# Makiato1999/HRI-EMO

Measured on AMD Instinct MI355X. Metric: utterances/sec fwd+bwd, d=768 T_a=400 T_t=128 N_e=6, higher is better.
Workload: dtype bf16; 1 GPU; FusionWithEmotionDecoder fwd+bwd (train mode, dropout 0.1), d=768 T_a=400 T_t=128 N_e=6 H=8, 2 fusion + 2 decoder layers, all-False masks (BASELINE cfg2); global_batch=64, batch_per_gpu=64, parallelism=dp1, grad_allreduce=none, launch=hipGraph replay, streams=2

## Files before the change

hri-emo_amd/csrc/attention.hip:

```cpp
#include <stdlib.h>

#include <type_traits>

#include "common.h"

struct AttnArgs {
  const bf16_t *Q, *K, *V;
  long ldq, ldk, ldv;
  bf16_t* O; long ldo;
  const bf16_t* dO; long lddo;
  bf16_t *dQ, *dK, *dV;
  long lddq, lddk, lddv;
  const uint8_t* kpm;
  float* lse;
  float* delta;
  float* probs;
  float* csq;
  float* cskv;
  int B, H, Lq, Lk;
  float scale;
  uint32_t thr16; float inv_keep; uint64_t seed; uint32_t site; int b_offset;
  float l2ik, keepfrac;
  const unsigned long long* seed_dev;
  unsigned long long* mbits;
// ... 1 lines not shown
  const int* cu_k;
  uint8_t* Oq; long ldoq;
  uint8_t* So; long ldso;
};

__device__ __forceinline__ AttnArgs localize(const AttnArgs& a0, int b, int h) {
  AttnArgs a = a0;
  if (a0.cu_q != nullptr) {
    const int q0 = a0.cu_q[b], k0 = a0.cu_k[b];
    const int Lq = a0.cu_q[b + 1] - q0, Lk = a0.cu_k[b + 1] - k0;
    const long sq = (long)q0 - (long)b * Lq, sk = (long)k0 - (long)b * Lk;
    a.Q += sq * a.ldq;
    if (a.O != nullptr) a.O += sq * a.ldo;
    if (a.dO != nullptr) a.dO += sq * a.lddo;
    if (a.dQ != nullptr) a.dQ += sq * a.lddq;
    a.K += sk * a.ldk;
    a.V += sk * a.ldv;
    if (a.dK != nullptr) a.dK += sk * a.lddk;
    if (a.dV != nullptr) a.dV += sk * a.lddv;
    const long bh = (long)b * a.H + h;
    if (a.lse != nullptr) a.lse += bh * (a0.Lq - Lq);
    if (a.delta != nullptr) a.delta += bh * (a0.Lq - Lq);
    if (a.mbits != nullptr) a.mbits += bh * ((long)a0.Lq * ((a0.Lk + 63) >> 6) - (long)Lq * ((Lk + 63) >> 6));
    a.Lq = Lq; a.Lk = Lk;
    a.kpm = nullptr;
  }
  return a;
}

#define EXP2(x) __builtin_amdgcn_exp2f(x)
#define LOG2E 1.4426950408889634f
#define LN2 0.6931471805599453f

template <int HD> struct AttnGeom {
  static constexpr int HDP = (HD + 31) / 32 * 32;
  static constexpr int KS = HDP / 32;
  static constexpr int DT = HD / 16;
  static constexpr int STRIDE = HDP * 2 + 32;
  static constexpr int CH = HD / 8;
  static constexpr int CHP = HDP / 8;
};

__device__ __forceinline__ bf16x8 zero8() {
  bf16x8 z;
#pragma unroll
  for (int i = 0; i < 8; ++i) z[i] = (bf16_t)0.f;
  return z;
}

__device__ __forceinline__ bf16x8 tr_frag(const char* tile, int stride, int row0, int col0, int lane) {
  const int g = lane >> 4, i = lane & 15;
  const char* a0 = tile + (row0 + 4 * g + (i >> 2)) * stride + (col0 + 4 * (i & 3)) * 2;
  s16x4 lo = __builtin_amdgcn_ds_read_tr16_b64_v4i16((LDS_PTR(s16x4))a0);
  s16x4 hi = __builtin_amdgcn_ds_read_tr16_b64_v4i16((LDS_PTR(s16x4))(a0 + 16 * stride));
  typedef __attribute__((ext_vector_type(8))) short s16x8;
  s16x8 r = {lo[0], lo[1], lo[2], lo[3], hi[0], hi[1], hi[2], hi[3]};
  return __builtin_bit_cast(bf16x8, r);
}
__device__ __forceinline__ bf16x8 row_frag(const char* tile, int stride, int row, int chunk) {
  return *(LDS_PTR(const bf16x8))(tile + row * stride + chunk * 16);
}

template <int HD, int NR, int NT>
__device__ __forceinline__ void load_tile(char* tile, const bf16_t* base, long ld, int row_first, int nrows_total, int tid) {
  using G = AttnGeom<HD>;
  for (int id = tid; id < NR * G::CHP; id += NT) {
// ... 22 lines not shown
    const u32x4_t v = __builtin_amdgcn_raw_buffer_load_b128(rsrc, ok ? (int)((r * ld + c * 8) * 2) : (int)0x80000000u, 0, 0);
    t.v[k] = __builtin_bit_cast(bf16x8, v);
  }
}
template <int HD, int NR, int NT>
__device__ __forceinline__ void tile_commit(const TileRegs<HD, NR, NT>& t, char* tile, int tid) {
  using G = AttnGeom<HD>;
#pragma unroll
  for (int k = 0; k < TileRegs<HD, NR, NT>::NPT; ++k) {
    const int id = tid + k * NT;
    const int r = id / G::CHP, c = id - r * G::CHP;
    if (id < NR * G::CHP) *(LDS_PTR(bf16x8))(tile + r * G::STRIDE + c * 16) = t.v[k];
  }
}

#ifndef DKV_QT
#define DKV_QT 32
#endif

__device__ __forceinline__ void tile_and_head(int ntiles, int nbh, int& tile, int& bh, int l = blockIdx.x) {
  const int full = (nbh >> 3) << 3;
  const int lim = full * ntiles;
  if (l < lim) {
    const int r = l >> 3;
    tile = r % ntiles;
    bh = (r / ntiles) * 8 + (l & 7);
  } else {
    const int r = l - lim;
    tile = r % ntiles;
    bh = full + r / ntiles;
  }
}

template <int HD, int NW, int QW, bool WB>
__global__ __launch_bounds__(NW * 64) void attn_fwd_kernel(const AttnArgs a0) {
  using G = AttnGeom<HD>;
  constexpr int KS = G::KS, DT = G::DT, STRIDE = G::STRIDE, NT = NW * 64;
  __shared__ __attribute__((aligned(16))) char lds[2 * 64 * STRIDE + 64 * 4 + 16];
  char* Kt = lds;
  char* Vt = lds + 64 * STRIDE;
  float* mb = (float*)(lds + 2 * 64 * STRIDE);
  int* padflag = (int*)(lds + 2 * 64 * STRIDE + 64 * 4);

  const int tid = threadIdx.x, lane = tid & 63, wave = tid >> 6, g = lane >> 4, i = lane & 15;
  int tile, bh;
  tile_and_head((a0.Lq + NW * QW * 16 - 1) / (NW * QW * 16), a0.B * a0.H, tile, bh);
  const int b = bh / a0.H, h = bh - b * a0.H;
  const AttnArgs a = localize(a0, b, h);
  if (tile * (NW * QW * 16) >= a.Lq) return;
  const int qbase = tile * (NW * QW * 16) + wave * QW * 16;

  bf16x8 qf[QW][KS];
#pragma unroll
  for (int qs = 0; qs < QW; ++qs) {
    const int qc = min(qbase + qs * 16 + i, a.Lq - 1);
    const bf16_t* qp = a.Q + ((long)b * a.Lq + qc) * a.ldq + h * HD;
#pragma unroll
    for (int ks = 0; ks < KS; ++ks) {
      const int e = ks * 32 + 8 * g;
      qf[qs][ks] = (e < HD) ? *(const bf16x8*)(qp + e) : zero8();
    }
  }
  f32x4 o[QW][DT];
  float m[QW], l[QW];
#pragma unroll
  for (int qs = 0; qs < QW; ++qs) {
    m[qs] = -INFINITY; l[qs] = 0.f;
#pragma unroll
    for (int dt = 0; dt < DT; ++dt) o[qs][dt] = (f32x4){0.f, 0.f, 0.f, 0.f};
  }
  const float sl2 = a.scale * LOG2E;
  const uint32_t key32 = site_key(eff_seed(a.seed, a.seed_dev), a.site, (uint32_t)((a.b_offset + b) * a.H + h));
  const bf16_t* Kb = a.K + (long)b * a.Lk * a.ldk + h * HD;
  const bf16_t* Vb = a.V + (long)b * a.Lk * a.ldv + h * HD;
  const int nkt = (a.Lk + 63) >> 6;

  constexpr bool PF = true;
  TileRegs<HD, 64, NT> kr, vr;
  if (PF) {
    tile_fetch<HD, 64, NT>(kr, Kb, a.ldk, 0, a.Lk, tid);
    tile_fetch<HD, 64, NT>(vr, Vb, a.ldv, 0, a.Lk, tid);
  }
  for (int kt = 0; kt < nkt; ++kt) {
    __syncthreads();
    if (PF) {
      tile_commit<HD, 64, NT>(kr, Kt, tid);
      tile_commit<HD, 64, NT>(vr, Vt, tid);
    } else {
      load_tile<HD, 64, NT>(Kt, Kb, a.ldk, kt * 64, a.Lk, tid);
      load_tile<HD, 64, NT>(Vt, Vb, a.ldv, kt * 64, a.Lk, tid);
    }
    if (tid < 64) {
      const int key = kt * 64 + tid;
      const bool pad = key >= a.Lk || (a.kpm != nullptr && a.kpm[(long)b * a.Lk + key] != 0);
      mb[tid] = pad ? -INFINITY : 0.f;
      const bool anyp = __builtin_amdgcn_ballot_w64(pad) != 0;
      if (tid == 0) padflag[0] = anyp ? 1 : 0;
    }
    __syncthreads();
    if (PF && kt + 1 < nkt) {
      tile_fetch<HD, 64, NT>(kr, Kb, a.ldk, (kt + 1) * 64, a.Lk, tid);
      tile_fetch<HD, 64, NT>(vr, Vb, a.ldv, (kt + 1) * 64, a.Lk, tid);
    }

    f32x4 s[QW][4];
#pragma unroll
    for (int qs = 0; qs < QW; ++qs)
#pragma unroll
      for (int n = 0; n < 4; ++n) s[qs][n] = (f32x4){0.f, 0.f, 0.f, 0.f};
#pragma unroll
    for (int n = 0; n < 4; ++n)
#pragma unroll
      for (int ks = 0; ks < KS; ++ks) {
        const bf16x8 kf = row_frag(Kt, STRIDE, n * 16 + i, ks * 4 + g);
#pragma unroll
        for (int qs = 0; qs < QW; ++qs) s[qs][n] = __builtin_amdgcn_mfma_f32_16x16x32_bf16(kf, qf[qs][ks], s[qs][n], 0, 0, 0);
      }

    const bool has_pad = padflag[0] != 0;
#pragma unroll
    for (int qs = 0; qs < QW; ++qs) {
      float mx = -INFINITY;
      if (has_pad) {
#pragma unroll
        for (int n = 0; n < 4; ++n) {
          const f32x4 bias = *(LDS_PTR(const f32x4))(mb + n * 16 + 4 * g);
#pragma unroll
          for (int r = 0; r < 4; ++r) s[qs][n][r] += bias[r];
        }
      }
#pragma unroll
      for (int n = 0; n < 4; ++n)
#pragma unroll
        for (int r = 0; r < 4; ++r) mx = fmaxf(mx, s[qs][n][r]);
      mx = fmaxf(mx, __shfl_xor(mx, 16));
      mx = fmaxf(mx, __shfl_xor(mx, 32));
      mx *= sl2;
      const float mnew = fmaxf(m[qs], mx);
      if (__builtin_amdgcn_ballot_w64(mnew > m[qs] + 8.f) != 0) {
        const float ms = (mnew == -INFINITY) ? 0.f : mnew;
        const float alpha = EXP2(m[qs] - ms);
        m[qs] = mnew;
        l[qs] *= alpha;
#pragma unroll
        for (int dt = 0; dt < DT; ++dt) o[qs][dt] *= alpha;
      }
      const float nm = (m[qs] == -INFINITY) ? 0.f : -m[qs];
      float rs = 0.f;
#pragma unroll
      for (int n = 0; n < 4; ++n)
#pragma unroll
        for (int r = 0; r < 4; ++r) {
          const float p = EXP2(fmaf(s[qs][n][r], sl2, nm));
          s[qs][n][r] = p;
          rs += p;
        }
      rs += __shfl_xor(rs, 16);
      rs += __shfl_xor(rs, 32);
      l[qs] += rs;
      if (a.thr16 != 0) {
        const uint32_t hb = drop_base(key32, (uint32_t)(qbase + qs * 16 + i), (uint32_t)((kt * 64 + 4 * g) >> 1));
        uint32_t bits = 0u;
#pragma unroll
        for (int n = 0; n < 4; ++n)
#pragma unroll
          for (int pr = 0; pr < 2; ++pr) {
            const uint32_t x = mix24(hb + (uint32_t)(n * 8 + pr) * DROP_CB);
            const bool k0 = keep_lo(x, a.thr16), k1 = keep_hi(x, a.thr16);
            s[qs][n][2 * pr] = k0 ? s[qs][n][2 * pr] : 0.f;
            s[qs][n][2 * pr + 1] = k1 ? s[qs][n][2 * pr + 1] : 0.f;
            if (WB) bits |= (k0 ? 1u : 0u) << (n * 4 + 2 * pr) | (k1 ? 1u : 0u) << (n * 4 + 2 * pr + 1);
          }
        if (WB && qbase + qs * 16 + i < a.Lq)
          ((unsigned short*)(a.mbits + (((long)bh * a.Lq + qbase + qs * 16 + i) * nkt + kt)))[g] = (unsigned short)bits;
      }
    }

#pragma unroll
    for (int s2 = 0; s2 < 2; ++s2) {
      bf16x8 pf[QW];
#pragma unroll
      for (int qs = 0; qs < QW; ++qs)
#pragma unroll
        for (int j = 0; j < 8; ++j) pf[qs][j] = (bf16_t)s[qs][2 * s2 + (j >> 2)][j & 3];
#pragma unroll
      for (int dt = 0; dt < DT; ++dt) {
        const bf16x8 vf = tr_frag(Vt, STRIDE, 32 * s2, dt * 16, lane);
#pragma unroll
        for (int qs = 0; qs < QW; ++qs) o[qs][dt] = __builtin_amdgcn_mfma_f32_16x16x32_bf16(vf, pf[qs], o[qs][dt], 0, 0, 0);
      }
    }
  }

#pragma unroll
  for (int qs = 0; qs < QW; ++qs) {
    const int q = qbase + qs * 16 + i;
    if (q >= a.Lq) continue;
    const float inv = (a.thr16 != 0 ? a.inv_keep : 1.f) / l[qs];
    bf16_t* op = a.O + ((long)b * a.Lq + q) * a.ldo + h * HD + 4 * g;
#pragma unroll
    for (int dt = 0; dt < DT; ++dt) {
      bf16x4 w;
#pragma unroll
      for (int r = 0; r < 4; ++r) w[r] = (bf16_t)(o[qs][dt][r] * inv);
      *(bf16x4*)(op + dt * 16) = w;
    }
    if (g == 0 && a.lse != nullptr) a.lse[((long)b * a.H + h) * a.Lq + q] = (m[qs] + log2f(l[qs])) * LN2;
  }
  if constexpr (DT % 2 == 0) {
    if (a.Oq != nullptr) {
#pragma unroll
      for (int qs = 0; qs < QW; ++qs) {
        const int q = qbase + qs * 16 + i;
        const float inv = (a.thr16 != 0 ? a.inv_keep : 1.f) / l[qs];
        const long row = (long)b * a.Lq + min(q, a.Lq - 1);
#pragma unroll
        for (int kb = 0; kb < DT / 2; ++kb) {
          float f[8];
          float amax = 0.f;
#pragma unroll
          for (int j = 0; j < 8; ++j) {
            f[j] = (float)(bf16_t)(o[qs][2 * kb + (j >> 2)][j & 3] * inv);
            amax = fmaxf(amax, fabsf(f[j]));
          }
          amax = fmaxf(amax, __shfl_xor(amax, 16));
// ... 82 lines not shown
        const bf16x8 ov = *(const bf16x8*)(op + e);
#pragma unroll
        for (int j = 0; j < 8; ++j) part += (float)dof[qs][ks][j] * (float)ov[j];
      } else {
        qf[qs][ks] = zero8();
        dof[qs][ks] = zero8();
      }
    }
    part += __shfl_xor(part, 16);
    part += __shfl_xor(part, 32);
    dl[qs] = part;
    const long li = ((long)b * a.H + h) * a.Lq + qc;
    lse2[qs] = a.lse[li] * LOG2E;
    if (g == 0 && q < a.Lq) a.delta[li] = part;
  }
  f32x4 dq[QW][DT];
#pragma unroll
  for (int qs = 0; qs < QW; ++qs)
#pragma unroll
    for (int dt = 0; dt < DT; ++dt) dq[qs][dt] = (f32x4){0.f, 0.f, 0.f, 0.f};

  const float sl2 = a.scale * LOG2E;
  float cexp[QW], dlk[QW];
#pragma unroll
  for (int qs = 0; qs < QW; ++qs) {
    cexp[qs] = (a.thr16 != 0 ? log2f(a.inv_keep) : 0.f) - lse2[qs];
    dlk[qs] = a.thr16 != 0 ? dl[qs] / a.inv_keep : dl[qs];
  }
  const uint32_t key32 = site_key(eff_seed(a.seed, a.seed_dev), a.site, (uint32_t)((a.b_offset + b) * a.H + h));
  const bf16_t* Kb = a.K + (long)b * a.Lk * a.ldk + h * HD;
  const bf16_t* Vb = a.V + (long)b * a.Lk * a.ldv + h * HD;
  const int nkt = (a.Lk + 63) >> 6;

  constexpr bool PF = (NW == 4);
  TileRegs<HD, 64, NT> kr, vr;
  if (PF) {
    tile_fetch<HD, 64, NT>(kr, Kb, a.ldk, 0, a.Lk, tid);
    tile_fetch<HD, 64, NT>(vr, Vb, a.ldv, 0, a.Lk, tid);
  }
  for (int kt = 0; kt < nkt; ++kt) {
    __syncthreads();
    if (PF) {
      tile_commit<HD, 64, NT>(kr, Kt, tid);
      tile_commit<HD, 64, NT>(vr, Vt, tid);
    } else {
      load_tile<HD, 64, NT>(Kt, Kb, a.ldk, kt * 64, a.Lk, tid);
      load_tile<HD, 64, NT>(Vt, Vb, a.ldv, kt * 64, a.Lk, tid);
    }
    if (tid < 64) {
      const int key = kt * 64 + tid;
      const bool pad = key >= a.Lk || (a.kpm != nullptr && a.kpm[(long)b * a.Lk + key] != 0);
      mb[tid] = pad ? -INFINITY : 0.f;
    }
    __syncthreads();
    if (PF && kt + 1 < nkt) {
      tile_fetch<HD, 64, NT>(kr, Kb, a.ldk, (kt + 1) * 64, a.Lk, tid);
      tile_fetch<HD, 64, NT>(vr, Vb, a.ldv, (kt + 1) * 64, a.Lk, tid);
    }

    f32x4 s[QW][4], dp[QW][4];
#pragma unroll
    for (int qs = 0; qs < QW; ++qs)
#pragma unroll
      for (int n = 0; n < 4; ++n) {
        s[qs][n] = (f32x4){0.f, 0.f, 0.f, 0.f};
        dp[qs][n] = (f32x4){0.f, 0.f, 0.f, 0.f};
      }
#pragma unroll
    for (int n = 0; n < 4; ++n)
#pragma unroll
      for (int ks = 0; ks < KS; ++ks) {
        const bf16x8 kf = row_frag(Kt, STRIDE, n * 16 + i, ks * 4 + g);
        const bf16x8 vf = row_frag(Vt, STRIDE, n * 16 + i, ks * 4 + g);
#pragma unroll
        for (int qs = 0; qs < QW; ++qs) {
          s[qs][n] = __builtin_amdgcn_mfma_f32_16x16x32_bf16(kf, qf[qs][ks], s[qs][n], 0, 0, 0);
          dp[qs][n] = __builtin_amdgcn_mfma_f32_16x16x32_bf16(vf, dof[qs][ks], dp[qs][n], 0, 0, 0);
        }
      }
#pragma unroll
    for (int qs = 0; qs < QW; ++qs) {
      const uint32_t hb = drop_base(key32, (uint32_t)(qbase + qs * 16 + i), (uint32_t)((kt * 64 + 4 * g) >> 1));
      uint32_t bits = 0xffffu;
      constexpr bool from_bits = BITS;
      if (from_bits && a.thr16 != 0)
        bits = ((const unsigned short*)(a.mbits + (((long)bh * a.Lq + min(qbase + qs * 16 + i, a.Lq - 1)) * nkt + kt)))[g];
#pragma unroll
      for (int n = 0; n < 4; ++n) {
        const f32x4 bias = *(LDS_PTR(const f32x4))(mb + n * 16 + 4 * g);
#pragma unroll
        for (int pr = 0; pr < 2; ++pr) {
          uint32_t x = 0xffffffffu;
          if (a.thr16 != 0 && !from_bits) x = mix24(hb + (uint32_t)(n * 8 + pr) * DROP_CB);
#pragma unroll
          for (int e = 0; e < 2; ++e) {
            const int r = 2 * pr + e;
            const float pk = EXP2(fmaf(s[qs][n][r], sl2, bias[r] + cexp[qs]));
            float dpd = dp[qs][n][r];
            if (a.thr16 != 0) {
              const bool keep = from_bits ? ((bits >> (n * 4 + r)) & 1u) != 0u : (e ? keep_hi(x, a.thr16) : keep_lo(x, a.thr16));
              dpd = keep ? dpd : 0.f;
            }
            s[qs][n][r] = pk * (dpd - dlk[qs]);
          }
        }
      }
    }
#pragma unroll
    for (int s2 = 0; s2 < 2; ++s2) {
      bf16x8 dsf[QW];
#pragma unroll
      for (int qs = 0; qs < QW; ++qs)
#pragma unroll
        for (int j = 0; j < 8; ++j) dsf[qs][j] = (bf16_t)s[qs][2 * s2 + (j >> 2)][j & 3];
#pragma unroll
      for (int dt = 0; dt < DT; ++dt) {
        const bf16x8 ktf = tr_frag(Kt, STRIDE, 32 * s2, dt * 16, lane);
#pragma unroll
        for (int qs = 0; qs < QW; ++qs) dq[qs][dt] = __builtin_amdgcn_mfma_f32_16x16x32_bf16(ktf, dsf[qs], dq[qs][dt], 0, 0, 0);
      }
    }
  }
  f32x4 cs[DT];
#pragma unroll
  for (int dt = 0; dt < DT; ++dt) cs[dt] = (f32x4){0.f, 0.f, 0.f, 0.f};
#pragma unroll
  for (int qs = 0; qs < QW; ++qs) {
    const int q = qbase + qs * 16 + i;
    if (q >= a.Lq) continue;
    bf16_t* dqp = a.dQ + ((long)b * a.Lq + q) * a.lddq + h * HD + 4 * g;
#pragma unroll
    for (int dt = 0; dt < DT; ++dt) {
      bf16x4 w;
#pragma unroll
      for (int r = 0; r < 4; ++r) {
        const float v = dq[qs][dt][r] * a.scale;
        w[r] = (bf16_t)v;
        cs[dt][r] += v;
      }
      *(bf16x4*)(dqp + dt * 16) = w;
    }
  }
  if (a.csq != nullptr) {
    __syncthreads();
    block_colsum_store<DT, NW>(cs, (float*)lds, csq_row, tid);
  }
}

template <int HD, bool BITS>
__global__ __launch_bounds__(512) void attn_bwd_qres_kernel(const AttnArgs a0) {
  using G = AttnGeom<HD>;
  constexpr int KS = G::KS, DT = G::DT, STRIDE = G::STRIDE, NW = 8, NT = 512, NQ = 128, KT = 64;
  constexpr int PS = KT * 2 + 32;
  __shared__ __attribute__((aligned(16))) char lds[2 * NQ * STRIDE + 2 * KT * STRIDE + 2 * NQ * PS + KT * 4];
  char* const Qi = lds;
// ... 184 lines not shown
      }
      *(bf16x4*)(dqp + dt * 16) = w;
    }
  }
  float* red = (float*)lds;
  if (a.csq != nullptr) {
    block_colsum_store<DT, NW>(csq, red, a.csq + (long)b * ((long)a.H * HD) + h * HD, tid);
    __syncthreads();
  }
  if (a.cskv != nullptr) {
#pragma unroll
    for (int dt = 0; dt < DT; ++dt) {
      f32x4 v = cs[dt];
#pragma unroll
      for (int m = 1; m < 16; m <<= 1) {
#pragma unroll
        for (int r = 0; r < 4; ++r) v[r] += __shfl_xor(v[r], m, 64);
      }
      if (i == 0) *(f32x4*)(red + wave * (DT * 16) + dt * 16 + 4 * g) = v;
    }
    __syncthreads();
    float* row = a.cskv + (long)b * (2L * a.H * HD) + h * HD;
    for (int c = tid; c < 2 * DT * 16; c += NT) {
      const int wh = c / (DT * 16), e = c - wh * (DT * 16);
      float t = 0.f;
#pragma unroll
      for (int w = 0; w < 4; ++w) t += red[(2 * w + (wh == 0 ? 1 : 0)) * (DT * 16) + e];
      row[(long)wh * a.H * HD + e] = t;
    }
  }
}

template <int HD, int NW, int KW, int QT>
__global__ __launch_bounds__(NW * 64) void attn_bwd_dkv_hash_kernel(const AttnArgs a0) {
  using G = AttnGeom<HD>;
  constexpr int KS = G::KS, DT = G::DT, STRIDE = G::STRIDE, NT = NW * 64;
  static_assert(QT == 32 || QT == 64, "query tile");
  constexpr int NQS = QT / 16, NKQ = QT / 32;
  constexpr int TILE_BYTES = 2 * QT * STRIDE + 2 * QT * 4;
  __shared__ __attribute__((aligned(16))) char lds[2 * TILE_BYTES];
  const int tid = threadIdx.x, lane = tid & 63, wave = tid >> 6, g = lane >> 4, i = lane & 15;
  int tile, bh;
  tile_and_head((a0.Lk + NW * KW * 16 - 1) / (NW * KW * 16), a0.B * a0.H, tile, bh);
  const int b = bh / a0.H, h = bh - b * a0.H;
  const AttnArgs a = localize(a0, b, h);
  float* const cskv_row = a.cskv != nullptr ? a.cskv + (long)(b * gridDim_tiles(a0.Lk, NW * KW * 16) + tile) * (2L * a.H * HD) + h * HD : nullptr;
  if (tile * (NW * KW * 16) >= a.Lk) {
    if (cskv_row != nullptr) for (int e = tid; e < HD; e += NT) { cskv_row[e] = 0.f; cskv_row[(long)a.H * HD + e] = 0.f; }
    return;
  }
  const int kbase = tile * (NW * KW * 16) + wave * KW * 16;

  bf16x8 kreg[KW][KS], vreg[KW][KS];
  bool kvalid[KW];
#pragma unroll
  for (int kw = 0; kw < KW; ++kw) {
    const int key = kbase + kw * 16 + i;
    const int kc = min(key, a.Lk - 1);
    kvalid[kw] = key < a.Lk && !(a.kpm != nullptr && a.kpm[(long)b * a.Lk + kc] != 0);
    const bf16_t* kp = a.K + ((long)b * a.Lk + kc) * a.ldk + h * HD;
    const bf16_t* vp = a.V + ((long)b * a.Lk + kc) * a.ldv + h * HD;
#pragma unroll
    for (int ks = 0; ks < KS; ++ks) {
      const int e = ks * 32 + 8 * g;
      kreg[kw][ks] = (e < HD) ? *(const bf16x8*)(kp + e) : zero8();
      vreg[kw][ks] = (e < HD) ? *(const bf16x8*)(vp + e) : zero8();
    }
// ... 10 lines not shown
      dv[kw][dt] = (f32x4){0.f, 0.f, 0.f, 0.f};
    }
  const float sl2 = a.scale * LOG2E;
  const uint32_t key32 = site_key(eff_seed(a.seed, a.seed_dev), a.site, (uint32_t)((a.b_offset + b) * a.H + h));
#pragma unroll
  for (int kw = 0; kw < KW; ++kw) hkb[kw] = drop_base(key32, 0u, (uint32_t)((kbase + kw * 16 + i) >> 1));
  const bf16_t* Qb = a.Q + (long)b * a.Lq * a.ldq + h * HD;
  const bf16_t* dOb = a.dO + (long)b * a.Lq * a.lddo + h * HD;
  const long lbase = ((long)b * a.H + h) * a.Lq;
  const int nqt = (a.Lq + QT - 1) / QT;

  const float l2ik = a.thr16 != 0 ? log2f(a.inv_keep) : 0.f, keepfrac = a.thr16 != 0 ? 1.f / a.inv_keep : 1.f;
  constexpr bool PF = (NW == 4);
  TileRegs<HD, QT, NT> qr, dor;
  float lse_r = 0.f, del_r = 0.f;
  auto fetch = [&](int qt) {
    tile_fetch<HD, QT, NT>(qr, Qb, a.ldq, qt * QT, a.Lq, tid);
    tile_fetch<HD, QT, NT>(dor, dOb, a.lddo, qt * QT, a.Lq, tid);
    if (tid < QT) {
      const int q = qt * QT + tid;
      lse_r = q < a.Lq ? l2ik - a.lse[lbase + q] * LOG2E : -INFINITY;
      del_r = q < a.Lq ? a.delta[lbase + q] * keepfrac : 0.f;
    }
  };
  auto commit = [&](int buf) {
    char* base = lds + buf * TILE_BYTES;
    tile_commit<HD, QT, NT>(qr, base, tid);
    tile_commit<HD, QT, NT>(dor, base + QT * STRIDE, tid);
    if (tid < QT) {
      ((float*)(base + 2 * QT * STRIDE))[tid] = lse_r;
      ((float*)(base + 2 * QT * STRIDE))[QT + tid] = del_r;
    }
  };
  fetch(0);
  commit(0);
  if (nqt > 1) fetch(1);
  __syncthreads();
  for (int qt = 0; qt < nqt; ++qt) {
    const char* Qt = lds + (qt & 1) * TILE_BYTES;
    const char* dOt = Qt + QT * STRIDE;
    const float* lse_s = (const float*)(Qt + 2 * QT * STRIDE);
    const float* del_s = lse_s + QT;
    if (qt + 1 < nqt) {
      commit((qt + 1) & 1);
      if (qt + 2 < nqt) fetch(qt + 2);
    }

    f32x4 s[KW][NQS], dp[KW][NQS];
#pragma unroll
    for (int kw = 0; kw < KW; ++kw)
#pragma unroll
      for (int qs = 0; qs < NQS; ++qs) {
        s[kw][qs] = (f32x4){0.f, 0.f, 0.f, 0.f};
        dp[kw][qs] = (f32x4){0.f, 0.f, 0.f, 0.f};
      }
#pragma unroll
    for (int qs = 0; qs < NQS; ++qs)
#pragma unroll
      for (int ks = 0; ks < KS; ++ks) {
        const bf16x8 qfr = row_frag(Qt, STRIDE, qs * 16 + i, ks * 4 + g);
        const bf16x8 dofr = row_frag(dOt, STRIDE, qs * 16 + i, ks * 4 + g);
#pragma unroll
        for (int kw = 0; kw < KW; ++kw) {
          s[kw][qs] = __builtin_amdgcn_mfma_f32_16x16x32_bf16(qfr, kreg[kw][ks], s[kw][qs], 0, 0, 0);
          dp[kw][qs] = __builtin_amdgcn_mfma_f32_16x16x32_bf16(dofr, vreg[kw][ks], dp[kw][qs], 0, 0, 0);
        }
      }
    bf16x8 pf[KW][NKQ], dsf[KW][NKQ];
#pragma unroll
    for (int qs = 0; qs < NQS; ++qs) {
      const f32x4 lse4 = *(LDS_PTR(const f32x4))(lse_s + qs * 16 + 4 * g);
      const f32x4 del4 = *(LDS_PTR(const f32x4))(del_s + qs * 16 + 4 * g);
#pragma unroll
      for (int kw = 0; kw < KW; ++kw) {
        const uint32_t key = (uint32_t)(kbase + kw * 16 + i);
#pragma unroll
        for (int r = 0; r < 4; ++r) {
          const float pk = kvalid[kw] ? EXP2(fmaf(s[kw][qs][r], sl2, lse4[r])) : 0.f;
          float pd = pk, dpd = dp[kw][qs][r];
          if (a.thr16 != 0) {
            const uint32_t x = mix24(hkb[kw] + (uint32_t)(qt * QT + qs * 16 + 4 * g + r) * DROP_CA);
            const bool keep = (key & 1u) ? keep_hi(x, a.thr16) : keep_lo(x, a.thr16);
            pd = keep ? pk : 0.f;
            dpd = keep ? dpd : 0.f;
          }
          pf[kw][qs >> 1][(qs & 1) * 4 + r] = (bf16_t)pd;
          dsf[kw][qs >> 1][(qs & 1) * 4 + r] = (bf16_t)(pk * (dpd - del4[r]));
        }
      }
    }
#pragma unroll
    for (int kq = 0; kq < NKQ; ++kq)
#pragma unroll
      for (int dt = 0; dt < DT; ++dt) {
        const bf16x8 dotf = tr_frag(dOt, STRIDE, 32 * kq, dt * 16, lane);
        const bf16x8 qtf = tr_frag(Qt, STRIDE, 32 * kq, dt * 16, lane);
#pragma unroll
        for (int kw = 0; kw < KW; ++kw) {
          dv[kw][dt] = __builtin_amdgcn_mfma_f32_16x16x32_bf16(dotf, pf[kw][kq], dv[kw][dt], 0, 0, 0);
          dk[kw][dt] = __builtin_amdgcn_mfma_f32_16x16x32_bf16(qtf, dsf[kw][kq], dk[kw][dt], 0, 0, 0);
        }
      }
    __syncthreads();
  }
  f32x4 csk[DT], csv[DT];
#pragma unroll
  for (int dt = 0; dt < DT; ++dt) { csk[dt] = (f32x4){0.f, 0.f, 0.f, 0.f}; csv[dt] = (f32x4){0.f, 0.f, 0.f, 0.f}; }
#pragma unroll
  for (int kw = 0; kw < KW; ++kw) {
    const int key = kbase + kw * 16 + i;
    if (key >= a.Lk) continue;
    bf16_t* dkp = a.dK + ((long)b * a.Lk + key) * a.lddk + h * HD + 4 * g;
    bf16_t* dvp = a.dV + ((long)b * a.Lk + key) * a.lddv + h * HD + 4 * g;
#pragma unroll
    for (int dt = 0; dt < DT; ++dt) {
      bf16x4 wk, wv;
#pragma unroll
      for (int r = 0; r < 4; ++r) {
        const float vk = dk[kw][dt][r] * a.scale, vv = dv[kw][dt][r];
        wk[r] = (bf16_t)vk;
        wv[r] = (bf16_t)vv;
        csk[dt][r] += vk;
        csv[dt][r] += vv;
      }
      *(bf16x4*)(dkp + dt * 16) = wk;
      *(bf16x4*)(dvp + dt * 16) = wv;
    }
  }
  if (a.cskv != nullptr) {
    float* row = cskv_row;
    __syncthreads();
    block_colsum_store<DT, NW>(csk, (float*)lds, row, tid);
    block_colsum_store<DT, NW>(csv, (float*)lds + NW * DT * 16, row + (long)a.H * HD, tid);
  }
}

template <int HD, int NW, int KW, int QT, bool BITS, bool FUSED, bool PACKED = false>
// ... 446 lines not shown
  HRIEMO_CHECK(hd == 16 || hd == 32 || hd == 64 || hd == 96 || hd == 128, "attn: head_dim %d not built (16/32/64/96/128)", hd);
  return 0;
}
static int check_common(const AttnArgs& a, int hd) {
  if (check_shape(a.B, a.H, a.Lq, a.Lk, hd)) return 1;
  HRIEMO_CHECK(a.ldq % 8 == 0 && a.ldk % 8 == 0 && a.ldv % 8 == 0, "attn: leading dims must be multiples of 8");
  HRIEMO_CHECK(((uintptr_t)a.Q % 16) == 0 && ((uintptr_t)a.K % 16) == 0 && ((uintptr_t)a.V % 16) == 0, "attn: unaligned Q/K/V");
  return 0;
}
static int check_packed(const AttnArgs& a) {
  HRIEMO_CHECK((a.cu_q == nullptr) == (a.cu_k == nullptr), "attn: cu_seqlens_q and cu_seqlens_k must be given together");
  HRIEMO_CHECK(a.cu_q == nullptr || a.kpm == nullptr, "attn: packed sequences carry their lengths, a key_padding_mask cannot be combined with them");
  return 0;
}

extern "C" int hriemo_attn_plan(int B, int H, int Lq, int Lk, int head_dim, int cus, int* fwd_rows, int* bwd_form, int* dq_rows,
                                int* dkv_rows, int* dq_colsum_rows, int* kv_colsum_rows) {
  HRIEMO_CHECK(fwd_rows != nullptr && bwd_form != nullptr && dq_rows != nullptr && dkv_rows != nullptr && dq_colsum_rows != nullptr &&
                   kv_colsum_rows != nullptr, "attn_plan: bad arguments");
  if (check_shape(B, H, Lq, Lk, head_dim)) return 1;
  const AttnPlan p = attn_plan(B, H, Lq, Lk, head_dim, cus);
  *fwd_rows = p.fwd_rows; *bwd_form = p.bwd_form; *dq_rows = p.dq_rows; *dkv_rows = p.dkv_rows;
  *dq_colsum_rows = p.dq_colsum_rows; *kv_colsum_rows = p.kv_colsum_rows;
  return 0;
}
extern "C" int hriemo_attn_bwd_single_pass(int B, int H, int Lk, int head_dim) { return attn_plan(B, H, 1, Lk, head_dim, 0).bwd_form == 1; }
extern "C" int hriemo_attn_bwd_single_pass_q(int B, int H, int Lq, int Lk, int head_dim) { return attn_plan(B, H, Lq, Lk, head_dim, 0).bwd_form != 0; }
extern "C" int hriemo_attn_bwd_kv_colsum_rows(int B, int H, int Lq, int Lk, int head_dim) { return attn_plan(B, H, Lq, Lk, head_dim, 0).kv_colsum_rows; }
extern "C" int hriemo_attn_bwd_colsum_rows(int B, int H, int L, int head_dim) { return attn_plan(B, H, 1, L, head_dim, 0).kv_colsum_rows; }
extern "C" int hriemo_attn_bwd_dq_colsum_rows(int B, int H, int Lq, int Lk, int head_dim) { return attn_plan(B, H, Lq, Lk, head_dim, 0).dq_colsum_rows; }

extern "C" long hriemo_attn_mask_bytes(int B, int H, int Lq, int Lk) { return (long)B * H * Lq * ((Lk + 63) / 64) * 8; }

template <int N> using Int = std::integral_constant<int, N>;
template <class F> static void with_head_dim(int head_dim, F&& f) {
  switch (head_dim) {
    case 16: f(Int<16>{}); break;
    case 32: f(Int<32>{}); break;
    case 64: f(Int<64>{}); break;
    case 96: f(Int<96>{}); break;
    case 128: f(Int<128>{}); break;
  }
}
template <class F> static void with_tile(int rows, F&& f) {
  if (rows == 128) f(Int<4>{}, Int<2>{});
  else if (rows == 64) f(Int<4>{}, Int<1>{});
  else f(Int<1>{}, Int<1>{});
}
template <class F> static void with_bool(bool v, F&& f) {
  if (v) f(std::true_type{});
  else f(std::false_type{});
}

static void fill_drop(AttnArgs& a, float p, uint64_t seed, const unsigned long long* seed_dev, uint32_t site, int b_offset) {
  DropCfg d = make_drop(p, seed, site);
  a.thr16 = d.thr16; a.inv_keep = d.inv_keep; a.seed = seed; a.site = site; a.b_offset = b_offset; a.seed_dev = seed_dev;
  a.l2ik = d.thr16 != 0 ? log2f(d.inv_keep) : 0.f;
  a.keepfrac = d.thr16 != 0 ? 1.f / d.inv_keep : 1.f;
}
static AttnArgs attn_args(const void* Q, long ldq, const void* K, long ldk, const void* V, long ldv, const unsigned char* key_padding_mask,
                          const float* lse, int B, int H, int Lq, int Lk, int head_dim, float p_drop, unsigned long long seed,
                          const unsigned long long* seed_dev, unsigned site, int b_offset) {
  AttnArgs a = {};
  a.Q = (const bf16_t*)Q; a.K = (const bf16_t*)K; a.V = (const bf16_t*)V;
  a.ldq = ldq; a.ldk = ldk; a.ldv = ldv;
  a.kpm = key_padding_mask; a.lse = (float*)lse; a.B = B; a.H = H; a.Lq = Lq; a.Lk = Lk;
  a.scale = 1.0f / sqrtf((float)head_dim);
// ... 177 lines not shown
```

Before: 8711 utterances/s.

## Specialize attention kernels for partial query/key tiles and set waves-per-EU hints

Attention fwd, bwd-dq and bwd-dkv kernels now split the inner loop into a full-tile path and a tail path instantiated at compile time. The tail path skips MFMA work on key or query sub-blocks past the sequence end, and waves whose rows fall entirely out of range only take part in the shared-memory staging and barriers. The forward and dkv kernels also gain amdgpu_waves_per_eu occupancy hints for some configurations. This trims wasted matrix work on ragged tiles (T_a=400 and T_t=128 are not all multiples of 64), at the cost of more code paths and possible register-pressure or code-size changes.

```diff
diff --git a/hri-emo_amd/csrc/attention.hip b/hri-emo_amd/csrc/attention.hip
--- a/hri-emo_amd/csrc/attention.hip
+++ b/hri-emo_amd/csrc/attention.hip
@@ -57,6 +57,8 @@
 #define LOG2E 1.4426950408889634f
 #define LN2 0.6931471805599453f
 
+template <int N> using Int = std::integral_constant<int, N>;
+
 template <int HD> struct AttnGeom {
   static constexpr int HDP = (HD + 31) / 32 * 32;
   static constexpr int KS = HDP / 32;
@@ -145,8 +147,14 @@
   }
 }
 
+template <int HD, int NW, int QW, bool WB> constexpr int fwd_waves() {
+  if (!WB) return 1;
+  if (NW == 1) return HD == 96 ? 2 : 1;
+  if (QW == 1 && HD == 16) return 6;
+  return ((QW == 1 && HD == 128) || (QW == 2 && HD == 64)) ? 3 : 1;
+}
 template <int HD, int NW, int QW, bool WB>
-__global__ __launch_bounds__(NW * 64) void attn_fwd_kernel(const AttnArgs a0) {
+__global__ __launch_bounds__(NW * 64) __attribute__((amdgpu_waves_per_eu(fwd_waves<HD, NW, QW, WB>()))) void attn_fwd_kernel(const AttnArgs a0) {
   using G = AttnGeom<HD>;
   constexpr int KS = G::KS, DT = G::DT, STRIDE = G::STRIDE, NT = NW * 64;
   __shared__ __attribute__((aligned(16))) char lds[2 * 64 * STRIDE + 64 * 4 + 16];
@@ -188,64 +196,48 @@
   const bf16_t* Vb = a.V + (long)b * a.Lk * a.ldv + h * HD;
   const int nkt = (a.Lk + 63) >> 6;
 
-  constexpr bool PF = true;
-  TileRegs<HD, 64, NT> kr, vr;
-  if (PF) {
-    tile_fetch<HD, 64, NT>(kr, Kb, a.ldk, 0, a.Lk, tid);
-    tile_fetch<HD, 64, NT>(vr, Vb, a.ldv, 0, a.Lk, tid);
-  }
-  for (int kt = 0; kt < nkt; ++kt) {
-    __syncthreads();
-    if (PF) {
-      tile_commit<HD, 64, NT>(kr, Kt, tid);
-      tile_commit<HD, 64, NT>(vr, Vt, tid);
-    } else {
-      load_tile<HD, 64, NT>(Kt, Kb, a.ldk, kt * 64, a.Lk, tid);
-      load_tile<HD, 64, NT>(Vt, Vb, a.ldv, kt * 64, a.Lk, tid);
-    }
-    if (tid < 64) {
-      const int key = kt * 64 + tid;
-      const bool pad = key >= a.Lk || (a.kpm != nullptr && a.kpm[(long)b * a.Lk + key] != 0);
-      mb[tid] = pad ? -INFINITY : 0.f;
-      const bool anyp = __builtin_amdgcn_ballot_w64(pad) != 0;
-      if (tid == 0) padflag[0] = anyp ? 1 : 0;
-    }
-    __syncthreads();
-    if (PF && kt + 1 < nkt) {
-      tile_fetch<HD, 64, NT>(kr, Kb, a.ldk, (kt + 1) * 64, a.Lk, tid);
-      tile_fetch<HD, 64, NT>(vr, Vb, a.ldv, (kt + 1) * 64, a.Lk, tid);
-    }
-
-    f32x4 s[QW][4];
-#pragma unroll
-    for (int qs = 0; qs < QW; ++qs)
+  constexpr bool SPEC = NW > 1 && !(WB && QW == 2 && (HD == 32 || HD == 64));
+  const int nq = SPEC ? min(QW, max(0, (a.Lq - (tile * (NW * QW * 16) + __builtin_amdgcn_readfirstlane(wave) * QW * 16) + 15) >> 4)) : QW;
+  const int kt_tail = (SPEC && (a.Lk & 63) != 0) ? nkt - 1 : nkt;
+  const int nv_tail = ((a.Lk & 63) + 15) >> 4;
+  auto tile_body = [&](auto nq_c, auto tail_c, const int kt, const int nv) __attribute__((always_inline)) {
+    constexpr int NQ = decltype(nq_c)::value;
+    constexpr bool TAIL = decltype(tail_c)::value;
+    f32x4 s[NQ][4];
+#pragma unroll
+    for (int qs = 0; qs < NQ; ++qs)
 #pragma unroll
       for (int n = 0; n < 4; ++n) s[qs][n] = (f32x4){0.f, 0.f, 0.f, 0.f};
 #pragma unroll
-    for (int n = 0; n < 4; ++n)
+    for (int n = 0; n < 4; ++n) {
+      if (TAIL && n >= nv) continue;
 #pragma unroll
       for (int ks = 0; ks < KS; ++ks) {
         const bf16x8 kf = row_frag(Kt, STRIDE, n * 16 + i, ks * 4 + g);
 #pragma unroll
-        for (int qs = 0; qs < QW; ++qs) s[qs][n] = __builtin_amdgcn_mfma_f32_16x16x32_bf16(kf, qf[qs][ks], s[qs][n], 0, 0, 0);
-      }
+        for (int qs = 0; qs < NQ; ++qs) s[qs][n] = __builtin_amdgcn_mfma_f32_16x16x32_bf16(kf, qf[qs][ks], s[qs][n], 0, 0, 0);
+      }
+    }
 
     const bool has_pad = padflag[0] != 0;
 #pragma unroll
-    for (int qs = 0; qs < QW; ++qs) {
+    for (int qs = 0; qs < NQ; ++qs) {
       float mx = -INFINITY;
       if (has_pad) {
 #pragma unroll
         for (int n = 0; n < 4; ++n) {
+          if (TAIL && n >= nv) continue;
           const f32x4 bias = *(LDS_PTR(const f32x4))(mb + n * 16 + 4 * g);
 #pragma unroll
           for (int r = 0; r < 4; ++r) s[qs][n][r] += bias[r];
         }
       }
 #pragma unroll
-      for (int n = 0; n < 4; ++n)
+      for (int n = 0; n < 4; ++n) {
+        if (TAIL && n >= nv) continue;
 #pragma unroll
         for (int r = 0; r < 4; ++r) mx = fmaxf(mx, s[qs][n][r]);
+      }
       mx = fmaxf(mx, __shfl_xor(mx, 16));
       mx = fmaxf(mx, __shfl_xor(mx, 32));
       mx *= sl2;
@@ -261,13 +253,15 @@
       const float nm = (m[qs] == -INFINITY) ? 0.f : -m[qs];
       float rs = 0.f;
 #pragma unroll
-      for (int n = 0; n < 4; ++n)
+      for (int n = 0; n < 4; ++n) {
+        if (TAIL && n >= nv) continue;
 #pragma unroll
         for (int r = 0; r < 4; ++r) {
           const float p = EXP2(fmaf(s[qs][n][r], sl2, nm));
           s[qs][n][r] = p;
           rs += p;
         }
+      }
       rs += __shfl_xor(rs, 16);
       rs += __shfl_xor(rs, 32);
       l[qs] += rs;
@@ -275,7 +269,8 @@
         const uint32_t hb = drop_base(key32, (uint32_t)(qbase + qs * 16 + i), (uint32_t)((kt * 64 + 4 * g) >> 1));
         uint32_t bits = 0u;
 #pragma unroll
-        for (int n = 0; n < 4; ++n)
+        for (int n = 0; n < 4; ++n) {
+          if (TAIL && n >= nv) continue;
 #pragma unroll
           for (int pr = 0; pr < 2; ++pr) {
             const uint32_t x = mix24(hb + (uint32_t)(n * 8 + pr) * DROP_CB);
@@ -284,6 +279,7 @@
             s[qs][n][2 * pr + 1] = k1 ? s[qs][n][2 * pr + 1] : 0.f;
             if (WB) bits |= (k0 ? 1u : 0u) << (n * 4 + 2 * pr) | (k1 ? 1u : 0u) << (n * 4 + 2 * pr + 1);
           }
+        }
         if (WB && qbase + qs * 16 + i < a.Lq)
           ((unsigned short*)(a.mbits + (((long)bh * a.Lq + qbase + qs * 16 + i) * nkt + kt)))[g] = (unsigned short)bits;
       }
@@ -291,19 +287,71 @@
 
 #pragma unroll
     for (int s2 = 0; s2 < 2; ++s2) {
-      bf16x8 pf[QW];
-#pragma unroll
-      for (int qs = 0; qs < QW; ++qs)
+      if (TAIL && 2 * s2 >= nv) continue;
+      bf16x8 pf[NQ];
+#pragma unroll
+      for (int qs = 0; qs < NQ; ++qs)
 #pragma unroll
         for (int j = 0; j < 8; ++j) pf[qs][j] = (bf16_t)s[qs][2 * s2 + (j >> 2)][j & 3];
 #pragma unroll
       for (int dt = 0; dt < DT; ++dt) {
         const bf16x8 vf = tr_frag(Vt, STRIDE, 32 * s2, dt * 16, lane);
 #pragma unroll
-        for (int qs = 0; qs < QW; ++qs) o[qs][dt] = __builtin_amdgcn_mfma_f32_16x16x32_bf16(vf, pf[qs], o[qs][dt], 0, 0, 0);
-      }
-    }
-  }
+        for (int qs = 0; qs < NQ; ++qs) o[qs][dt] = __builtin_amdgcn_mfma_f32_16x16x32_bf16(vf, pf[qs], o[qs][dt], 0, 0, 0);
+      }
+    }
+  };
+
+  constexpr bool PF = true;
+  TileRegs<HD, 64, NT> kr, vr;
+  if (PF) {
+    tile_fetch<HD, 64, NT>(kr, Kb, a.ldk, 0, a.Lk, tid);
+    tile_fetch<HD, 64, NT>(vr, Vb, a.ldv, 0, a.Lk, tid);
+  }
+  auto stage = [&](const int kt) __attribute__((always_inline)) {
+    __syncthreads();
+    if (PF) {
+      tile_commit<HD, 64, NT>(kr, Kt, tid);
+      tile_commit<HD, 64, NT>(vr, Vt, tid);
+    } else {
+      load_tile<HD, 64, NT>(Kt, Kb, a.ldk, kt * 64, a.Lk, tid);
+      load_tile<HD, 64, NT>(Vt, Vb, a.ldv, kt * 64, a.Lk, tid);
+    }
+    if (tid < 64) {
+      const int key = kt * 64 + tid;
+      const bool pad = key >= a.Lk || (a.kpm != nullptr && a.kpm[(long)b * a.Lk + key] != 0);
+      mb[tid] = pad ? -INFINITY : 0.f;
+      const bool anyp = __builtin_amdgcn_ballot_w64(pad) != 0;
+      if (tid == 0) padflag[0] = anyp ? 1 : 0;
+    }
+    __syncthreads();
+    if (PF && kt + 1 < nkt) {
+      tile_fetch<HD, 64, NT>(kr, Kb, a.ldk, (kt + 1) * 64, a.Lk, tid);
+      tile_fetch<HD, 64, NT>(vr, Vb, a.ldv, (kt + 1) * 64, a.Lk, tid);
+    }
+  };
+  auto sweep = [&](auto nq_c) __attribute__((always_inline)) {
+    constexpr int NQ = decltype(nq_c)::value;
+    if constexpr (NQ == QW) {
+      for (int kt = 0; kt < kt_tail; ++kt) {
+        stage(kt);
+        tile_body(nq_c, std::false_type{}, kt, 4);
+      }
+      if (kt_tail < nkt) {
+        stage(kt_tail);
+        tile_body(nq_c, std::true_type{}, kt_tail, nv_tail);
+      }
+    } else {
+      for (int kt = 0; kt < nkt; ++kt) {
+        stage(kt);
+        if constexpr (NQ > 0) tile_body(nq_c, std::true_type{}, kt, kt != kt_tail ? 4 : nv_tail);
+      }
+    }
+  };
+  constexpr bool HALF = QW > 1 && !WB;
+  if (nq == QW || (!HALF && nq > 0)) sweep(Int<QW>{});
+  else if (HALF && nq == 1) sweep(Int<HALF ? 1 : 0>{});
+  else sweep(Int<0>{});
 
 #pragma unroll
   for (int qs = 0; qs < QW; ++qs) {
@@ -452,54 +500,37 @@
   const bf16_t* Vb = a.V + (long)b * a.Lk * a.ldv + h * HD;
   const int nkt = (a.Lk + 63) >> 6;
 
-  constexpr bool PF = (NW == 4);
-  TileRegs<HD, 64, NT> kr, vr;
-  if (PF) {
-    tile_fetch<HD, 64, NT>(kr, Kb, a.ldk, 0, a.Lk, tid);
-    tile_fetch<HD, 64, NT>(vr, Vb, a.ldv, 0, a.Lk, tid);
-  }
-  for (int kt = 0; kt < nkt; ++kt) {
-    __syncthreads();
-    if (PF) {
-      tile_commit<HD, 64, NT>(kr, Kt, tid);
-      tile_commit<HD, 64, NT>(vr, Vt, tid);
-    } else {
-      load_tile<HD, 64, NT>(Kt, Kb, a.ldk, kt * 64, a.Lk, tid);
-      load_tile<HD, 64, NT>(Vt, Vb, a.ldv, kt * 64, a.Lk, tid);
-    }
-    if (tid < 64) {
-      const int key = kt * 64 + tid;
-      const bool pad = key >= a.Lk || (a.kpm != nullptr && a.kpm[(long)b * a.Lk + key] != 0);
-      mb[tid] = pad ? -INFINITY : 0.f;
-    }
-    __syncthreads();
-    if (PF && kt + 1 < nkt) {
-      tile_fetch<HD, 64, NT>(kr, Kb, a.ldk, (kt + 1) * 64, a.Lk, tid);
-      tile_fetch<HD, 64, NT>(vr, Vb, a.ldv, (kt + 1) * 64, a.Lk, tid);
-    }
-
-    f32x4 s[QW][4], dp[QW][4];
-#pragma unroll
-    for (int qs = 0; qs < QW; ++qs)
+  constexpr bool SPEC = QW == 1 && NW > 1;
+  const int nq = SPEC ? min(QW, max(0, (a.Lq - (tile * (NW * QW * 16) + __builtin_amdgcn_readfirstlane(wave) * QW * 16) + 15) >> 4)) : QW;
+  const int kt_tail = (SPEC && (a.Lk & 63) != 0) ? nkt - 1 : nkt;
+  const int nv_tail = ((a.Lk & 63) + 15) >> 4;
+  auto tile_body = [&](auto nq_c, auto tail_c, const int kt, const int nv) __attribute__((always_inline)) {
+    constexpr int NQ = decltype(nq_c)::value;
+    constexpr bool TAIL = decltype(tail_c)::value;
+    f32x4 s[NQ][4], dp[NQ][4];
+#pragma unroll
+    for (int qs = 0; qs < NQ; ++qs)
 #pragma unroll
       for (int n = 0; n < 4; ++n) {
         s[qs][n] = (f32x4){0.f, 0.f, 0.f, 0.f};
         dp[qs][n] = (f32x4){0.f, 0.f, 0.f, 0.f};
       }
 #pragma unroll
-    for (int n = 0; n < 4; ++n)
+    for (int n = 0; n < 4; ++n) {
+      if (TAIL && n >= nv) continue;
 #pragma unroll
       for (int ks = 0; ks < KS; ++ks) {
         const bf16x8 kf = row_frag(Kt, STRIDE, n * 16 + i, ks * 4 + g);
         const bf16x8 vf = row_frag(Vt, STRIDE, n * 16 + i, ks * 4 + g);
 #pragma unroll
-        for (int qs = 0; qs < QW; ++qs) {
+        for (int qs = 0; qs < NQ; ++qs) {
           s[qs][n] = __builtin_amdgcn_mfma_f32_16x16x32_bf16(kf, qf[qs][ks], s[qs][n], 0, 0, 0);
           dp[qs][n] = __builtin_amdgcn_mfma_f32_16x16x32_bf16(vf, dof[qs][ks], dp[qs][n], 0, 0, 0);
         }
       }
-#pragma unroll
-    for (int qs = 0; qs < QW; ++qs) {
+    }
+#pragma unroll
+    for (int qs = 0; qs < NQ; ++qs) {
       const uint32_t hb = drop_base(key32, (uint32_t)(qbase + qs * 16 + i), (uint32_t)((kt * 64 + 4 * g) >> 1));
       uint32_t bits = 0xffffu;
       constexpr bool from_bits = BITS;
@@ -507,6 +538,7 @@
         bits = ((const unsigned short*)(a.mbits + (((long)bh * a.Lq + min(qbase + qs * 16 + i, a.Lq - 1)) * nkt + kt)))[g];
 #pragma unroll
       for (int n = 0; n < 4; ++n) {
+        if (TAIL && n >= nv) continue;
         const f32x4 bias = *(LDS_PTR(const f32x4))(mb + n * 16 + 4 * g);
 #pragma unroll
         for (int pr = 0; pr < 2; ++pr) {
@@ -528,19 +560,64 @@
     }
 #pragma unroll
     for (int s2 = 0; s2 < 2; ++s2) {
-      bf16x8 dsf[QW];
-#pragma unroll
-      for (int qs = 0; qs < QW; ++qs)
+      if (TAIL && 2 * s2 >= nv) continue;
+      bf16x8 dsf[NQ];
+#pragma unroll
+      for (int qs = 0; qs < NQ; ++qs)
 #pragma unroll
         for (int j = 0; j < 8; ++j) dsf[qs][j] = (bf16_t)s[qs][2 * s2 + (j >> 2)][j & 3];
 #pragma unroll
       for (int dt = 0; dt < DT; ++dt) {
         const bf16x8 ktf = tr_frag(Kt, STRIDE, 32 * s2, dt * 16, lane);
 #pragma unroll
-        for (int qs = 0; qs < QW; ++qs) dq[qs][dt] = __builtin_amdgcn_mfma_f32_16x16x32_bf16(ktf, dsf[qs], dq[qs][dt], 0, 0, 0);
-      }
-    }
-  }
+        for (int qs = 0; qs < NQ; ++qs) dq[qs][dt] = __builtin_amdgcn_mfma_f32_16x16x32_bf16(ktf, dsf[qs], dq[qs][dt], 0, 0, 0);
+      }
+    }
+  };
+
+  constexpr bool PF = (NW == 4);
+  TileRegs<HD, 64, NT> kr, vr;
+  if (PF) {
+    tile_fetch<HD, 64, NT>(kr, Kb, a.ldk, 0, a.Lk, tid);
+    tile_fetch<HD, 64, NT>(vr, Vb, a.ldv, 0, a.Lk, tid);
+  }
+  auto stage = [&](const int kt) __attribute__((always_inline)) {
+    __syncthreads();
+    if (PF) {
+      tile_commit<HD, 64, NT>(kr, Kt, tid);
+      tile_commit<HD, 64, NT>(vr, Vt, tid);
+    } else {
+      load_tile<HD, 64, NT>(Kt, Kb, a.ldk, kt * 64, a.Lk, tid);
+      load_tile<HD, 64, NT>(Vt, Vb, a.ldv, kt * 64, a.Lk, tid);
+    }
+    if (tid < 64) {
+      const int key = kt * 64 + tid;
+      const bool pad = key >= a.Lk || (a.kpm != nullptr && a.kpm[(long)b * a.Lk + key] != 0);
+      mb[tid] = pad ? -INFINITY : 0.f;
+    }
+    __syncthreads();
+    if (PF && kt + 1 < nkt) {
+      tile_fetch<HD, 64, NT>(kr, Kb, a.ldk, (kt + 1) * 64, a.Lk, tid);
+      tile_fetch<HD, 64, NT>(vr, Vb, a.ldv, (kt + 1) * 64, a.Lk, tid);
+    }
+  };
+  auto sweep = [&](auto nq_c) __attribute__((always_inline)) {
+    constexpr int NQ = decltype(nq_c)::value;
+    if constexpr (NQ == QW) {
+      for (int kt = 0; kt < kt_tail; ++kt) {
+        stage(kt);
+        tile_body(nq_c, std::false_type{}, kt, 4);
+      }
+      if (kt_tail < nkt) {
+        stage(kt_tail);
+        tile_body(nq_c, std::true_type{}, kt_tail, nv_tail);
+      }
+    } else {
+      for (int kt = 0; kt < nkt; ++kt) stage(kt);
+    }
+  };
+  if (nq == QW) sweep(Int<QW>{});
+  else sweep(Int<0>{});
   f32x4 cs[DT];
 #pragma unroll
   for (int dt = 0; dt < DT; ++dt) cs[dt] = (f32x4){0.f, 0.f, 0.f, 0.f};
@@ -791,7 +868,7 @@
 }
 
 template <int HD, int NW, int KW, int QT>
-__global__ __launch_bounds__(NW * 64) void attn_bwd_dkv_hash_kernel(const AttnArgs a0) {
+__global__ __launch_bounds__(NW * 64) __attribute__((amdgpu_waves_per_eu((HD == 32 && NW == 4 && KW == 1) ? 5 : 1))) void attn_bwd_dkv_hash_kernel(const AttnArgs a0) {
   using G = AttnGeom<HD>;
   constexpr int KS = G::KS, DT = G::DT, STRIDE = G::STRIDE, NT = NW * 64;
   static_assert(QT == 32 || QT == 64, "query tile");
@@ -868,47 +945,53 @@
       ((float*)(base + 2 * QT * STRIDE))[QT + tid] = del_r;
     }
   };
-  fetch(0);
-  commit(0);
-  if (nqt > 1) fetch(1);
-  __syncthreads();
-  for (int qt = 0; qt < nqt; ++qt) {
+  constexpr bool SPEC = KW == 1 && NW > 1;
+  const int nk = SPEC ? min(KW, max(0, (a.Lk - (tile * (NW * KW * 16) + __builtin_amdgcn_readfirstlane(wave) * KW * 16) + 15) >> 4)) : KW;
+  const int qt_tail = (SPEC && (a.Lq % QT) != 0) ? nqt - 1 : nqt;
+  const int nqs_tail = ((a.Lq % QT) + 15) >> 4;
+  auto tile_body = [&](auto nk_c, auto tail_c, const int qt, const int nqs) __attribute__((always_inline)) {
+    constexpr int NK = decltype(nk_c)::value;
+    constexpr bool TAIL = decltype(tail_c)::value;
     const char* Qt = lds + (qt & 1) * TILE_BYTES;
     const char* dOt = Qt + QT * STRIDE;
     const float* lse_s = (const float*)(Qt + 2 * QT * STRIDE);
     const float* del_s = lse_s + QT;
-    if (qt + 1 < nqt) {
-      commit((qt + 1) & 1);
-      if (qt + 2 < nqt) fetch(qt + 2);
-    }
-
-    f32x4 s[KW][NQS], dp[KW][NQS];
-#pragma unroll
-    for (int kw = 0; kw < KW; ++kw)
+    f32x4 s[NK][NQS], dp[NK][NQS];
+#pragma unroll
+    for (int kw = 0; kw < NK; ++kw)
 #pragma unroll
       for (int qs = 0; qs < NQS; ++qs) {
         s[kw][qs] = (f32x4){0.f, 0.f, 0.f, 0.f};
         dp[kw][qs] = (f32x4){0.f, 0.f, 0.f, 0.f};
       }
 #pragma unroll
-    for (int qs = 0; qs < NQS; ++qs)
+    for (int qs = 0; qs < NQS; ++qs) {
+      if (TAIL && qs >= nqs) continue;
 #pragma unroll
       for (int ks = 0; ks < KS; ++ks) {
         const bf16x8 qfr = row_frag(Qt, STRIDE, qs * 16 + i, ks * 4 + g);
         const bf16x8 dofr = row_frag(dOt, STRIDE, qs * 16 + i, ks * 4 + g);
 #pragma unroll
-        for (int kw = 0; kw < KW; ++kw) {
+        for (int kw = 0; kw < NK; ++kw) {
           s[kw][qs] = __builtin_amdgcn_mfma_f32_16x16x32_bf16(qfr, kreg[kw][ks], s[kw][qs], 0, 0, 0);
           dp[kw][qs] = __builtin_amdgcn_mfma_f32_16x16x32_bf16(dofr, vreg[kw][ks], dp[kw][qs], 0, 0, 0);
         }
       }
-    bf16x8 pf[KW][NKQ], dsf[KW][NKQ];
+    }
+    bf16x8 pf[NK][NKQ], dsf[NK][NKQ];
+    if (TAIL) {
+#pragma unroll
+      for (int kw = 0; kw < NK; ++kw)
+#pragma unroll
+        for (int kq = 0; kq < NKQ; ++kq) { pf[kw][kq] = zero8(); dsf[kw][kq] = zero8(); }
+    }
 #pragma unroll
     for (int qs = 0; qs < NQS; ++qs) {
+      if (TAIL && qs >= nqs) continue;
       const f32x4 lse4 = *(LDS_PTR(const f32x4))(lse_s + qs * 16 + 4 * g);
       const f32x4 del4 = *(LDS_PTR(const f32x4))(del_s + qs * 16 + 4 * g);
 #pragma unroll
-      for (int kw = 0; kw < KW; ++kw) {
+      for (int kw = 0; kw < NK; ++kw) {
         const uint32_t key = (uint32_t)(kbase + kw * 16 + i);
 #pragma unroll
         for (int r = 0; r < 4; ++r) {
@@ -926,19 +1009,52 @@
       }
     }
 #pragma unroll
-    for (int kq = 0; kq < NKQ; ++kq)
+    for (int kq = 0; kq < NKQ; ++kq) {
+      if (TAIL && 2 * kq >= nqs) continue;
 #pragma unroll
       for (int dt = 0; dt < DT; ++dt) {
         const bf16x8 dotf = tr_frag(dOt, STRIDE, 32 * kq, dt * 16, lane);
         const bf16x8 qtf = tr_frag(Qt, STRIDE, 32 * kq, dt * 16, lane);
 #pragma unroll
-        for (int kw = 0; kw < KW; ++kw) {
+        for (int kw = 0; kw < NK; ++kw) {
           dv[kw][dt] = __builtin_amdgcn_mfma_f32_16x16x32_bf16(dotf, pf[kw][kq], dv[kw][dt], 0, 0, 0);
           dk[kw][dt] = __builtin_amdgcn_mfma_f32_16x16x32_bf16(qtf, dsf[kw][kq], dk[kw][dt], 0, 0, 0);
         }
       }
-    __syncthreads();
-  }
+    }
+  };
+  fetch(0);
+  commit(0);
+  if (nqt > 1) fetch(1);
+  __syncthreads();
+  auto stage = [&](const int qt) __attribute__((always_inline)) {
+    if (qt + 1 < nqt) {
+      commit((qt + 1) & 1);
+      if (qt + 2 < nqt) fetch(qt + 2);
+    }
+  };
+  auto sweep = [&](auto nk_c) __attribute__((always_inline)) {
+    constexpr int NK = decltype(nk_c)::value;
+    if constexpr (NK == KW) {
+      for (int qt = 0; qt < qt_tail; ++qt) {
+        stage(qt);
+        tile_body(nk_c, std::false_type{}, qt, NQS);
+        __syncthreads();
+      }
+      if (qt_tail < nqt) {
+        stage(qt_tail);
+        tile_body(nk_c, std::true_type{}, qt_tail, nqs_tail);
+        __syncthreads();
+      }
+    } else {
+      for (int qt = 0; qt < nqt; ++qt) {
+        stage(qt);
+        __syncthreads();
+      }
+    }
+  };
+  if (nk == KW) sweep(Int<KW>{});
+  else sweep(Int<0>{});
   f32x4 csk[DT], csv[DT];
 #pragma unroll
   for (int dt = 0; dt < DT; ++dt) { csk[dt] = (f32x4){0.f, 0.f, 0.f, 0.f}; csv[dt] = (f32x4){0.f, 0.f, 0.f, 0.f}; }
@@ -1451,7 +1567,6 @@
 
 extern "C" long hriemo_attn_mask_bytes(int B, int H, int Lq, int Lk) { return (long)B * H * Lq * ((Lk + 63) / 64) * 8; }
 
-template <int N> using Int = std::integral_constant<int, N>;
 template <class F> static void with_head_dim(int head_dim, F&& f) {
   switch (head_dim) {
     case 16: f(Int<16>{}); break;
```

Result: no change. 8704 utterances/s (median of 5 runs) (-0.1%).
